# Koellewe/nano-dpow

Measured on AMD Instinct MI355X. Metric: Gnonce/s blake2b-64 per GPU & 8-GPU node; p50 time-to-work at fffffff8, higher is better.
Workload: dtype u64

## Files before the change

### include/nanopow.h

```cpp
#ifndef NANOPOW_H
#define NANOPOW_H

#include <stdint.h>

#ifdef __cplusplus
extern "C" {
#endif

#define NPOW_OK 0
#define NPOW_CANCELLED 1
#define NPOW_EXHAUSTED 2
#define NPOW_PENDING 3
#define NPOW_TOO_LATE 4
#define NPOW_ERR_NOT_INITIALISED (-1)
#define NPOW_ERR_NO_DEVICE (-2)
#define NPOW_ERR_BAD_ARGUMENT (-3)
#define NPOW_ERR_HIP (-4)
#define NPOW_ERR_INVALID_WORK (-5)
#define NPOW_ERR_CAPACITY (-6)
#define NPOW_ERR_INTERNAL (-7)

#define NPOW_ABI_VERSION 7

#define NPOW_RESERVE_MIN 0xfffff00000000000ull
// ... 165 lines not shown
  uint64_t nonces_done;
  uint64_t nonce, value;
  uint64_t launches;
  uint64_t records;
  uint64_t records_max;
  uint64_t room;
} npow_best_info;

int npow_ticket_best(uint64_t ticket, npow_best_info* out);

int npow_submit_best_background(const uint8_t root[32], uint64_t floor, uint64_t start, uint64_t count,
                                uint64_t device_mask, const volatile uint32_t* cancel, uint64_t* ticket);

typedef struct npow_best_hold_info {
  uint32_t size;
  uint32_t background;
  uint64_t launches_cut;
  uint64_t held_us;
} npow_best_hold_info;

int npow_ticket_best_hold(uint64_t ticket, npow_best_hold_info* out);

int npow_submit_sweep_shared(const uint8_t root[32], uint64_t threshold, uint64_t start, uint64_t count,
                             uint64_t device_mask, const volatile uint32_t* cancel, uint64_t* ticket);
int npow_submit_best_shared(const uint8_t root[32], uint64_t floor, uint64_t start, uint64_t count,
                            uint64_t device_mask, const volatile uint32_t* cancel, uint64_t* ticket);

typedef struct npow_range_share_info {
  uint32_t size;
  uint32_t klass;
  uint64_t launches;
  uint64_t launches_cut;
  uint64_t held_us;
  uint64_t moves;
} npow_range_share_info;

int npow_ticket_share(uint64_t ticket, npow_range_share_info* out);

int npow_values(int device, const uint8_t root[32], uint64_t start, uint64_t count, uint64_t* values_out);

int npow_values_path(int device, const uint8_t root[32], uint64_t start, uint64_t count, int path,
                     uint64_t* values_out);

int npow_values_pairs(int device, const uint8_t* roots, const uint64_t* nonces, uint32_t n,
                      uint64_t* values_out);

int npow_set_tuning(uint32_t iters_per_launch, uint32_t poll_interval, uint32_t blocks_per_cu);

int npow_set_pool_tuning(uint32_t budget_us, uint32_t blocks_per_cu);

int npow_device_stats_get(int device, npow_device_stats* out);
int npow_device_stats_get_sized(int device, npow_device_stats* out, uint64_t size);
int npow_device_stats_reset(int device);

const char* npow_version(void);
int npow_abi_version(void);

#ifdef __cplusplus
}
#endif

#endif
```

### nano-dpow_amd/csrc/npow_engine.cpp

```cpp
#include <hip/hip_runtime.h>

#include <pthread.h>
#include <time.h>

#include <algorithm>
#include <cstddef>
#include <exception>
#include <chrono>
#include <cstdio>
#include <cstdlib>
#include <cstring>
#include <deque>
#include <memory>
#include <mutex>
#include <string>
#include <thread>
#include <vector>

#include "npow_host.h"

namespace npow {

namespace {
thread_local std::string t_err;
// ... 475 lines not shown
  out->host_cpu_ms = cpu - d.worker_cpu0_ms;
  out->host_wall_ms = std::chrono::duration<double, std::milli>(std::chrono::steady_clock::now() - d.stats_t0).count();
  out->dead = d.dead ? 1 : 0;
  out->pool_groups = kLsGroups;
  out->early_finishes = d.early;
  out->early_mismatches = d.early_mismatch;
  out->yields = d.yields;
  out->dyn_entries = d.dyn;
  out->kills_relayed = d.kills_relayed;
  out->late_nonces = d.late;
  out->hip_device = d.hip_id;
  out->cu_first = d.cu_first;
  out->idle_ms = d.idle_ms;
  out->idle_gaps = d.idle_gaps;
  out->affinity_checks = d.affinity_checks.load(std::memory_order_relaxed);
  out->affinity_failures = d.affinity_failures.load(std::memory_order_relaxed);
  out->watcher_decisions = d.watcher_decisions;
  out->stale_drains = d.stale_drains;
  out->linger_relays = d.linger_relays;
  out->stale_late = d.stale_late;
  out->stale_missing = d.stale_missing;
  out->stale_gpu_delay_us = d.stale_gpu_delay_us;
  out->linger_ms = d.linger_ms;
  out->promotions = d.promotions;
  return NPOW_OK;
}

int npow_device_stats_get(int device, npow_device_stats* out) try {
  if (!out) return fail(NPOW_ERR_BAD_ARGUMENT, "out is required");
  npow_device_stats full;
  if (int rc = stats_fill(device, &full)) return rc;
  memcpy(out, &full, offsetof(npow_device_stats, kills_relayed));
  return NPOW_OK;
} catch (...) { return guard_exception(); }

int npow_device_stats_get_sized(int device, npow_device_stats* out, uint64_t size) try {
  if (!out || size == 0) return fail(NPOW_ERR_BAD_ARGUMENT, "out and size > 0 are required");
  npow_device_stats full;
  if (int rc = stats_fill(device, &full)) return rc;
  memcpy(out, &full, std::min<uint64_t>(size, sizeof(full)));
  return NPOW_OK;
} catch (...) { return guard_exception(); }

int npow_device_stats_reset(int device) try {
  if (int rc = check_init()) return rc;
  if (device < 0 || device >= (int)g_devs.size()) return fail(NPOW_ERR_BAD_ARGUMENT, "bad device");
  Device& d = *g_devs[device];
  settle_stats(d);
  const double cpu = worker_cpu_ms(d);
  std::lock_guard<std::mutex> g(d.stats_mu);
  d.launches = d.nonces = d.invalid = d.early = d.early_mismatch = d.yields = d.dyn = d.kills_relayed = d.late = 0;
  d.promotions = d.idle_gaps = d.watcher_decisions = d.stale_drains = d.linger_relays = d.stale_late = d.stale_missing = 0;
  d.idle_ms = d.linger_ms = d.stale_gpu_delay_us = 0.0;
  d.kernel_ms = 0.0;
  d.clk_ticks = d.clk_ref_ticks = 0.0;
  d.stats_t0 = std::chrono::steady_clock::now();
  d.worker_cpu0_ms = cpu;
  return NPOW_OK;
} catch (...) { return guard_exception(); }

int npow_search(const uint8_t root[32], uint64_t threshold, uint64_t start, uint64_t device_mask,
                uint64_t max_nonces_per_device, const volatile uint32_t* cancel, uint64_t* nonce_out,
                uint64_t* value_out, uint64_t* nonces_done) try {
  if (int rc = check_init()) return rc;
  if (!root || !nonce_out) return fail(NPOW_ERR_BAD_ARGUMENT, "root and nonce_out are required");
  uint64_t ticket = 0;
  if (int rc = pool_submit(root, threshold, start, device_mask, max_nonces_per_device, cancel, &ticket)) return rc;
  return pool_wait(ticket, -1, nonce_out, value_out, nonces_done);
} catch (...) { return guard_exception(); }

int npow_search_batch(const uint8_t* roots, const uint64_t* thresholds, uint32_t n, uint64_t device_mask,
                      uint64_t max_nonces_per_root, const volatile uint32_t* const* cancel, uint64_t* nonces_out,
                      uint64_t* values_out, int32_t* status_out, uint64_t* nonces_done) try {
  if (int rc = check_init()) return rc;
  if (nonces_done) *nonces_done = 0;
  if (n == 0) return NPOW_OK;
  if (!roots || !thresholds || !nonces_out || !status_out)
    return fail(NPOW_ERR_BAD_ARGUMENT, "roots, thresholds, nonces_out and status_out are required");
  std::vector<uint64_t> tickets(n, 0);
  int err = NPOW_OK;
  std::string err_msg;
  for (uint32_t i = 0; i < n; ++i) {
    const uint8_t* r = roots + 32 * (size_t)i;
    const uint64_t start = host_load_le64(r) ^ host_load_le64(r + 24);
    int rc = pool_submit(r, thresholds[i], start, device_mask, max_nonces_per_root, cancel ? cancel[i] : nullptr,
                         &tickets[i]);
    if (rc) {
      status_out[i] = rc;
      if (err == NPOW_OK) {
        err = rc;
        err_msg = last_error();
      }
    }
  }
  uint64_t total = 0;
  for (uint32_t i = 0; i < n; ++i) {
    if (!tickets[i]) continue;
    uint64_t nonce = 0, value = 0, done = 0;
    const int rc = pool_wait(tickets[i], -1, &nonce, &value, &done);
    total += done;
    status_out[i] = rc;
    if (rc == NPOW_OK) {
      nonces_out[i] = nonce;
      if (values_out) values_out[i] = value;
    } else if (rc < 0 && err == NPOW_OK) {
      err = rc;
      err_msg = last_error();
    }
  }
  if (nonces_done) *nonces_done = total;
  if (err != NPOW_OK) return fail(err, err_msg);
// ... 370 lines not shown
```

### nano-dpow_amd/csrc/npow_host.h

```cpp
#pragma once
#include <hip/hip_runtime.h>
#include <pthread.h>

#include <atomic>
#include <condition_variable>
#include <chrono>
#include <memory>
#include <mutex>
#include <string>
#include <thread>
#include <vector>

#include "../../include/nanopow.h"
#include "npow_blake2b.h"
#include "npow_internal.h"

namespace npow {

int fail(int code, const std::string& msg);
const std::string& last_error();

#define HIPTRY(expr)                                                                        \
  do {                                                                                      \
    hipError_t e_ = (expr);                                                                 \
    if (e_ != hipSuccess)                                                                   \
      return ::npow::fail(NPOW_ERR_HIP, std::string(#expr) + ": " + hipGetErrorString(e_)); \
  } while (0)

constexpr int kEventRing = 4;
static_assert(kEventRing == sizeof(PoolMailbox::clk) / sizeof(PoolMailbox::clk[0]), "one clock record set per ring");

struct Device {
  int id = 0;
  int cpu_threads = 0;
  int hip_id = 0;
  int cus = 0;
  bool time_shared = false;
  int cu_first = -1;
  hipStream_t stream = nullptr;
  DevState* st = nullptr;
  HostMailbox* mb = nullptr;
  HostMailbox* mb_dev = nullptr;
  uint64_t* d_out = nullptr;
  hipEvent_t ev_start[kEventRing] = {};
  hipEvent_t ev_stop[kEventRing] = {};
  std::mutex mu;
  std::atomic<int> tasks_waiting{0};
  PoolDevState* pst = nullptr;
  PoolMailbox* pmb = nullptr;
  PoolMailbox* pmb_dev = nullptr;
  PoolTable* d_tab[kEventRing] = {};
  PoolTable* h_tab[kEventRing] = {};
  unsigned long long* h_done = nullptr;
  hipEvent_t ev_done[kMaxSlots] = {};
  hipStream_t hit_stream = nullptr;
  unsigned long long* h_hit_ring = nullptr;
  unsigned long long* h_hit_n = nullptr;
  uint64_t* h_hits = nullptr;
  std::thread worker;
  std::mutex stats_mu;
  uint64_t launches = 0, nonces = 0, invalid = 0;
  uint64_t early = 0, early_mismatch = 0;
  uint64_t yields = 0, dyn = 0;
  uint64_t linger_ends = 0;
  uint64_t promotions = 0;
  std::atomic<int> counted_inflight{0};
  uint64_t kills_relayed = 0;
  uint64_t late = 0;
  uint64_t watcher_decisions = 0;
  uint64_t stale_drains = 0;
  uint64_t stale_late = 0;
  uint64_t stale_missing = 0;
  double stale_gpu_delay_us = 0.0;
  uint64_t linger_relays = 0;
  double linger_ms = 0.0;
  double idle_ms = 0.0;
  uint64_t idle_gaps = 0;
  std::atomic<bool> worker_busy{false};
  std::atomic<int> active_slots{0};
  std::mutex wake_mu;
  std::condition_variable wake_cv;
  uint64_t wake_seq = 0;
  std::atomic<uint64_t> armed_mask{0};
  std::atomic<uint64_t> armed_gen[kMaxSlots] = {};
  std::atomic<const volatile uint32_t*> armed_cancel[kMaxSlots] = {};
  std::atomic<double> armed_spin_until[kMaxSlots] = {};
  std::mutex armed_mu;
  std::shared_ptr<void> armed_job[kMaxSlots];
  double kernel_ms = 0.0;
  double clk_ticks = 0.0, clk_ref_ticks = 0.0;
  std::chrono::steady_clock::time_point stats_t0 = std::chrono::steady_clock::now();
  double worker_cpu0_ms = 0.0;
  std::atomic<bool> dead{false};
  int dead_code = NPOW_ERR_HIP;
  std::string dead_msg;
  std::atomic<uint64_t> affinity_checks{0}, affinity_failures{0};
  std::mutex cpu_tids_mu;
  std::vector<pthread_t> cpu_tids;
};

extern std::vector<std::unique_ptr<Device>> g_devs;
extern std::atomic<uint32_t> g_iters;
extern std::atomic<uint32_t> g_poll;
extern std::atomic<uint32_t> g_blocks_per_cu;
extern std::atomic<uint32_t> g_budget_us;

inline int grid_of(const Device& d) { return d.cus * (int)g_blocks_per_cu.load(); }
inline int ls_grid(const Device& d) { return d.cus * kLsGroups; }
inline PoolShape pool_shape(const Device& d) { return PoolShape{ls_grid(d)}; }
inline uint32_t poll_mask() {
  uint32_t p = g_poll.load();
  uint32_t m = 1;
  while (m < p) m <<= 1;
  return m - 1;
}

// ... 81 lines not shown
```

### nano-dpow_amd/csrc/npow_internal.h

```cpp
#pragma once
#include <stddef.h>
#include <stdint.h>
#include <hip/hip_runtime.h>

#include "npow_blake2b.h"
#include "npow_weights.h"
#include "npow_claims.h"
#include "npow_dense.h"
#include "npow_hash_asm.inc"
#include "npow_hash_asm_lockstep_ld.inc"

namespace npow {

constexpr int kBlock = 256;
constexpr int kLsWaves = 8;
constexpr int kLsBlock = kLsWaves * 64;
static_assert(kDenseWaves == (uint32_t)kLsWaves, "npow_dense.h: one block per wave of a workgroup");
constexpr int kLsGroups = 4;

enum class Mode : int { kSweep = 1, kValues = 2, kValuesSeq = 3 };

struct LaunchArgs {
  uint64_t u[NPOW_ASM_N_UNIFORMS];
  uint64_t threshold;
// ... 153 lines not shown
  uint64_t t_fin;
  uint64_t t_relay;
  uint64_t t_join;
  uint64_t linger_gen;
  uint64_t stale;
};
static_assert(sizeof(PoolFin) == 64, "one line per slot");
struct alignas(16) PoolFloor {
  uint64_t threshold;
  uint64_t gen;
};
struct alignas(16) PoolReserve {
  uint64_t gen;
  uint64_t nonce;
};
constexpr int kDynEntries = 32;
constexpr int kDynRing = 2 * kDynEntries;
struct alignas(64) PoolDynEntry {
  PoolEntry e;
};
static_assert(sizeof(PoolDynEntry) == 192, "3 cache lines per dynamic entry");
struct PoolMailbox {
  PoolWin win[kMaxSlots];
  PoolFin fin[kMaxSlots];
  PoolDynEntry dyn[kDynRing];
  uint64_t kill[kMaxSlots];
  uint64_t boost[kMaxSlots];
  PoolFloor floor[kMaxSlots];
  PoolReserve reserve[kMaxSlots];
  alignas(64) uint64_t ctl;
  alignas(64) uint64_t kills;
  alignas(64) PoolClk clk[kPoolRing][kClkWaves];
#ifdef NPOW_DIAG_TIMES
  uint64_t diag_join[1024];
#endif
};

struct PoolShape {
  int grid;
  uint32_t units() const { return (uint32_t)grid; }
  uint64_t own(uint32_t e, uint32_t n, uint32_t iters) const {
    return dense_own(units(), n, e, iters);
  }
  uint64_t full(uint32_t iters) const { return dense_full(units(), iters); }
  uint32_t launch_iters(uint32_t iters) const { return iters > 1 ? iters / 2 : 1u; }
};

hipError_t launch_task(Mode mode, int grid, hipStream_t stream, const LaunchArgs& a, DevState* st,
                       HostMailbox* mb, uint64_t* out);
hipError_t launch_pool(hipStream_t stream, int grid, const PoolTable* tab, bool bounded, PoolDevState* st,
                       PoolMailbox* mb);
hipError_t launch_pool_arg(hipStream_t stream, int grid, const PoolTable& host_tab, bool bounded, PoolDevState* st,
                           PoolMailbox* mb);
inline void fill_uniforms(LaunchArgs& a, const RootPrecomp& pre) { npow_asm_uniforms(pre.m, a.u); }

hipError_t launch_pairs(int grid, hipStream_t stream, const uint64_t* roots_words, const uint64_t* nonces,
                        uint32_t n, uint64_t* out);

}
```

### nano-dpow_amd/csrc/npow_kernel.hip

```cpp
#include <hip/hip_runtime.h>
#include <stdint.h>
#include <string.h>

#include "npow_internal.h"

namespace npow {

__device__ __forceinline__ uint64_t pack(uint32_t lo, uint32_t hi) { return ((uint64_t)hi << 32) | lo; }

__device__ __forceinline__ uint64_t rotr32(uint64_t x) {
  return pack((uint32_t)(x >> 32), (uint32_t)x);
}
template <int N>
__device__ __forceinline__ uint64_t rotr_lt32(uint64_t x) {
  const uint32_t lo = (uint32_t)x, hi = (uint32_t)(x >> 32);
  return pack(__builtin_amdgcn_alignbit(hi, lo, N), __builtin_amdgcn_alignbit(lo, hi, N));
}
__device__ __forceinline__ uint64_t rotr63(uint64_t x) {
  const uint32_t lo = (uint32_t)x, hi = (uint32_t)(x >> 32);
  return pack(__builtin_amdgcn_alignbit(lo, hi, 31), __builtin_amdgcn_alignbit(hi, lo, 31));
}

template <int I>
__device__ __forceinline__ uint64_t add_msg(uint64_t a, uint64_t nonce, const uint64_t (&m)[4]) {
// ... 1021 lines not shown
    }
    __syncthreads();
    e = __builtin_amdgcn_readfirstlane(__hip_atomic_load(&s_next, __ATOMIC_RELAXED, __HIP_MEMORY_SCOPE_WORKGROUP));
    ++seg;
  }
  if constexpr (BOUNDED) {
    if (e != kNoEntry || !counted) break;
    __syncthreads();
    if (wv == 0) {
      const uint32_t next = ls2_move_claimed(tab, st, mb, (uint32_t)t_start);
      if (lane == 0) s_next = next;
    }
    __syncthreads();
    e = __builtin_amdgcn_readfirstlane(__hip_atomic_load(&s_next, __ATOMIC_RELAXED, __HIP_MEMORY_SCOPE_WORKGROUP));
    if (e == kNoEntry) break;
    continue;
  }
  if (e != kNoEntry || !tab->linger) break;
  __syncthreads();
  if (wv == 0) {
    const uint32_t next = ls2_linger(tab, st, mb, &s_seen, 0);
    if (lane == 0) s_next = next;
  }
  __syncthreads();
  e = __builtin_amdgcn_readfirstlane(__hip_atomic_load(&s_next, __ATOMIC_RELAXED, __HIP_MEMORY_SCOPE_WORKGROUP));
  if (e == kNoEntry) break;
  }
  if (!counted && wv == 0) ls2_exit(tab, st, mb, G, g);
  clk_end_ls2(tab, mb, t_start, wv);
}

template <bool BOUNDED>
__global__ __launch_bounds__(kLsBlock, 8) void npow_pool_kernel_ls2(const PoolTable* __restrict__ tab,
                                                                   PoolDevState* __restrict__ st,
                                                                   PoolMailbox* __restrict__ mb) {
  uint64_t t_start;
  asm volatile("s_memrealtime %0\n\ts_waitcnt lgkmcnt(0)" : "=s"(t_start) :: "memory");
  clk_begin_lds();
  pool_body_ls2<BOUNDED>(tab, st, mb, t_start);
}

template <bool BOUNDED>
__global__ __launch_bounds__(kLsBlock, 8) void npow_pool_kernel_ls2_arg(const PoolTableArg targ,
                                                                       PoolDevState* __restrict__ st,
                                                                       PoolMailbox* __restrict__ mb) {
  uint64_t t_start;
  asm volatile("s_memrealtime %0\n\ts_waitcnt lgkmcnt(0)" : "=s"(t_start) :: "memory");
  (void)targ;
  const PoolTable* tab = (const PoolTable*)__builtin_amdgcn_kernarg_segment_ptr();
  clk_begin_lds();
  pool_body_ls2<BOUNDED>(tab, st, mb, t_start);
}

hipError_t launch_pool(hipStream_t stream, int grid, const PoolTable* tab, bool bounded, PoolDevState* st,
                       PoolMailbox* mb) {
  if (bounded)
    npow_pool_kernel_ls2<true><<<grid, kLsBlock, 0, stream>>>(tab, st, mb);
  else
    npow_pool_kernel_ls2<false><<<grid, kLsBlock, 0, stream>>>(tab, st, mb);
  return hipGetLastError();
}

hipError_t launch_pool_arg(hipStream_t stream, int grid, const PoolTable& host_tab, bool bounded, PoolDevState* st,
                           PoolMailbox* mb) {
  if (host_tab.n > (uint32_t)kArgEntries) return hipErrorInvalidValue;
  PoolTableArg a;
  memcpy(&a, &host_tab, pool_table_bytes(host_tab.n));
  if (bounded)
    npow_pool_kernel_ls2_arg<true><<<grid, kLsBlock, 0, stream>>>(a, st, mb);
  else
    npow_pool_kernel_ls2_arg<false><<<grid, kLsBlock, 0, stream>>>(a, st, mb);
  return hipGetLastError();
}

__global__ __launch_bounds__(kBlock) void npow_pairs_kernel(const uint64_t* __restrict__ roots_words,
                                                            const uint64_t* __restrict__ nonces, uint32_t n,
                                                            uint64_t* __restrict__ out) {
  const uint32_t i = blockIdx.x * kBlock + threadIdx.x;
  if (i >= n) return;
  uint64_t m[4];
#pragma unroll
  for (int k = 0; k < 4; ++k) m[k] = roots_words[4 * (size_t)i + k];
  out[i] = work_value_full(nonces[i], m);
}

hipError_t launch_task(Mode mode, int grid, hipStream_t stream, const LaunchArgs& a, DevState* st,
                       HostMailbox* mb, uint64_t* out) {
  switch (mode) {
    case Mode::kSweep:
      npow_sweep_kernel_ls2<<<grid, kLsBlock, 0, stream>>>(a, st, mb, out);
      break;
    case Mode::kValues:
      npow_values_kernel_ls2<<<grid, kLsBlock, 0, stream>>>(a, st, out);
      break;
    case Mode::kValuesSeq:
      npow_values_kernel_seq<<<grid, kBlock, 0, stream>>>(a, st, out);
      break;
  }
  return hipGetLastError();
}

hipError_t launch_pairs(int grid, hipStream_t stream, const uint64_t* roots_words, const uint64_t* nonces,
                        uint32_t n, uint64_t* out) {
  npow_pairs_kernel<<<grid, kBlock, 0, stream>>>(roots_words, nonces, n, out);
  return hipGetLastError();
}
// ... 3 lines not shown
```

### nano-dpow_amd/csrc/npow_pool.cpp

```cpp
#include <hip/hip_runtime.h>
#include <sys/prctl.h>

#include <algorithm>
#include <chrono>
#include <cmath>
#include <condition_variable>
#include <deque>
#include <mutex>
#include <string>
#include <thread>
#include <vector>

#include "npow_pool_impl.h"

namespace npow {
namespace {

constexpr double kYieldMinUs = 1500.0;
constexpr int kYieldMaxLive = 8;
constexpr int kIdleSpinUs = 2000;
constexpr double kPrelaunchUs = 2000.0;
constexpr double kDynMinUs = 3000.0;
constexpr double kFreshSpinUs = 400.0;
constexpr int kInvalidStreakMax = 3;
// ... 904 lines not shown
  bool fg = foreground_live(-1);
  for (uint32_t e = 0; e < n && !fg; ++e) fg = !slots_[idx[e]].job->background && !slots_[idx[e]].job->shared;
  const double t = now_us();
  uint32_t m = 0;
  for (uint32_t e = 0; e < n; ++e) {
    Slot& sl = slots_[idx[e]];
    if (!sl.job->held_class()) {
      idx[m++] = idx[e];
      continue;
    }
    JobDev& jd = sl.job->dev[sl.k];
    if (fg) {
      if (!sl.held) jd.held_since = t;
      sl.held = true;
      continue;
    }
    if (sl.held) {
      jd.held_us += t - jd.held_since;
      jd.held_since = 0;
      sl.held = false;
    }
    idx[m++] = idx[e];
  }
  return m;
}

int Worker::launch(bool empty_linger) {
  if (q_.size() >= 2 || d_.dead) return NPOW_OK;
  if (q_.size() == 1 && g_budget_us.load() > 0 && budget_left_us() > kPrelaunchUs && live_slot()) return NPOW_OK;
  uint32_t n = 0;
  int idx[kMaxSlots];
  bool claimed = false;
  for (int s = 0; s < kMaxSlots; ++s)
    if (slots_[s].state == SlotState::kActive && !slots_[s].no_more) {
      idx[n++] = s;
      claimed = claimed || slots_[s].job->held_class();
    }
  if (claimed) n = hold_out(idx, n);
  if (n == 0 && !empty_linger) return NPOW_OK;
  if (!live_slot()) end_linger();
  PoolTable& t = *d_.h_tab[ring_];
  bool bounded = false;
  build_table(t, idx, n, &bounded);
  if (n == 0 && !t.linger) return NPOW_OK;
  const PoolShape sh = pool_shape(d_);
  const int r = ring_;
  ring_ = (ring_ + 1) % kEventRing;
  const size_t bytes = pool_table_bytes(n);
  DEVCHECK(d_, "pool launch");
  if (faults().hip_dev == d_.id && seq_ > faults().hip_after)
    return fail(NPOW_ERR_HIP, "injected launch failure (NANOPOW_FAULT_HIP)");
  if (!collect_.empty())
    HIPTRY(hipMemsetAsync(&d_.pst->hits[r & 1], 0, offsetof(PoolHits, rec), d_.stream));
  if (n <= (uint32_t)kArgEntries) {
    HIPTRY(hipEventRecord(d_.ev_start[r], d_.stream));
    HIPTRY(launch_pool_arg(d_.stream, sh.grid, t, bounded, d_.pst, d_.pmb_dev));
  } else {
    HIPTRY(hipMemcpyAsync(d_.d_tab[r], d_.h_tab[r], bytes, hipMemcpyHostToDevice, d_.stream));
    HIPTRY(hipEventRecord(d_.ev_start[r], d_.stream));
    HIPTRY(launch_pool(d_.stream, sh.grid, d_.d_tab[r], bounded, d_.pst, d_.pmb_dev));
  }
  if (!collect_.empty())
    HIPTRY(hipMemcpyAsync(d_.h_hit_ring + (size_t)r * (offsetof(PoolHits, rec) / sizeof(unsigned long long)),
                          &d_.pst->hits[r & 1], offsetof(PoolHits, rec), hipMemcpyDeviceToHost, d_.stream));
  HIPTRY(hipEventRecord(d_.ev_stop[r], d_.stream));
  if (q_.empty()) front_start_ = std::chrono::steady_clock::now();
  NPOW_DBGT("nanopow[%d]: launch %llu n=%u linger %u wsum %u (weights halved %u times) yield_base %llx slots:", d_.id,
            (unsigned long long)seq_, n, t.linger, t.wsum ? t.wsum : pool_claimed_pad_sum(t.pad), t.wdown, (unsigned long long)t.yield_base);
  for (uint32_t e = 0; e < n; ++e) NPOW_DBG(" %d/g%llu", idx[e], (unsigned long long)t.e[e].gen);
  NPOW_DBG("\n");
  q_.push_back({seq_, r, (uint32_t)ctl_, t.yield_base, t.counted != 0, t.linger != 0, t.wdown, bounded, collect_});
  publish_counted();
  return NPOW_OK;
}

int Worker::queue_readbacks() {
  constexpr size_t row = kPoolDoneShards * 8;
  DEVCHECK(d_, "pool read-back");
  for (int s = 0; s < kMaxSlots; ++s) {
    Slot& sl = slots_[s];
    if (sl.state != SlotState::kDraining || sl.readback || sl.no_readback) continue;
    if (!g_readback_always && !d_.dead) {
      if (sl.early) {
        if (++early_count_ % kVerifyEvery != 0) {
          sl.no_readback = true;
          continue;
        }
      } else if (!sl.fin_seen && sl.stop_us > 0 && !sl.requeue && !sl.inflight.empty() &&
                 now_us() - sl.stop_us < g_linger_us) {
        continue;
      }
    }
    HIPTRY(hipMemcpyAsync(d_.h_done + (size_t)s * row, &d_.pst->done[s][0], row * sizeof(unsigned long long),
                          hipMemcpyDeviceToHost, d_.stream));
    HIPTRY(hipEventRecord(d_.ev_done[s], d_.stream));
    sl.readback = true;
  }
  return NPOW_OK;
}

void Worker::trace_launch(const PoolInflight& f, uint64_t g0, uint64_t g1) {
  float ev = 0.f;
  if (hipEventElapsedTime(&ev, d_.ev_start[f.ring], d_.ev_stop[f.ring]) == hipSuccess)
    fprintf(stderr, "nanopow-launch dev %d launch %llu: events %.1f clock waves %.1f us, start %.1f us after the "
            "previous end\n", d_.id, (unsigned long long)f.seq, ev * 1e3, (double)(g1 - g0) / 100.0,
            prev_g1_ ? ((double)g0 - (double)prev_g1_) / 100.0 : -1.0);
  prev_g1_ = g1;
// ... 502 lines not shown
```

### nano-dpow_amd/csrc/npow_pool_impl.h

```cpp
#pragma once
#include <cstdio>
#include <cstdlib>
#include <cstring>

#include "npow_pool.h"

namespace npow {

inline const char* env_str(const char* name, const char* dflt) { const char* e = getenv(name); return e ? e : dflt; }
inline double env_num(const char* name, double dflt) { const char* e = getenv(name); return e ? atof(e) : dflt; }
inline const double g_poll_us = env_num("NANOPOW_POLL_US", 50.0);
inline const bool g_debug = getenv("NANOPOW_DEBUG") != nullptr;
inline const int g_linger_env = getenv("NANOPOW_LINGER") ? (getenv("NANOPOW_LINGER")[0] == '0' ? 0 : 1) : -1;
inline const uint32_t g_linger_p = [] {
  uint32_t p = (uint32_t)atoi(env_str("NANOPOW_LINGER_P", "0")), q = 1;
  while (p && q < p) q <<= 1;
  return p ? q : 0u;
}();
inline const double g_linger_us = env_num("NANOPOW_LINGER_US", 1000.0);
inline const bool g_readback_always = strcmp(env_str("NANOPOW_READBACK", ""), "always") == 0;
inline const bool g_watcher_on = strcmp(env_str("NANOPOW_WATCHER", "1"), "0") != 0;
inline const double g_watch_nap_us = env_num("NANOPOW_WATCH_NAP_US", 20.0);
inline const bool g_trace_lat = getenv("NANOPOW_TRACE_LATENCY") != nullptr;
inline const bool g_trace_steps = getenv("NANOPOW_TRACE_STEPS") != nullptr;
inline const bool g_wait_spin = env_str("NANOPOW_WAIT_SPIN", "1")[0] != '0';

struct Faults {
  uint64_t invalid_mask = 0;
  int hip_dev = -1;
  uint64_t hip_after = 0;
  bool retarget_blind = false;
  bool no_moves = false;
};
const Faults& faults();

#define NPOW_DBG(...) \
  do { if (g_debug) fprintf(stderr, __VA_ARGS__); } while (0)
#define NPOW_DBGT(...) \
  do { if (g_debug) fprintf(stderr, "[%.3f] ", now_us() * 1e-3), fprintf(stderr, __VA_ARGS__); } while (0)

void wake_worker(Device& d);


inline void mb_kill(Device& d, int s, uint64_t gen) {
  __atomic_store_n(&d.pmb->kill[s], gen, __ATOMIC_RELEASE);
  __atomic_fetch_add(&d.pmb->kills, 1ull, __ATOMIC_RELEASE);
}
inline void mb_boost(Device& d, int s, uint64_t gen, uint32_t weight) {
  __atomic_store_n(&d.pmb->boost[s], pool_boost_word(gen, pool_wsh(weight)), __ATOMIC_RELEASE);
  __atomic_fetch_add(&d.pmb->kills, 1ull << 32, __ATOMIC_RELEASE);
}
inline void mb_floor(Device& d, int s, uint64_t gen, uint64_t threshold) {
  PoolFloor& f = d.pmb->floor[s];
  if (__atomic_load_n(&f.gen, __ATOMIC_RELAXED) != gen) {
    __atomic_store_n(&f.threshold, threshold, __ATOMIC_RELAXED);
    __atomic_store_n(&f.gen, gen, __ATOMIC_RELEASE);
  } else {
    __atomic_store_n(&f.threshold, threshold, __ATOMIC_RELEASE);
  }
}
inline void mb_yield(Device& d, uint64_t& ctl) {
  ctl += 1ull << 32;
  __atomic_store_n(&d.pmb->ctl, ctl, __ATOMIC_RELEASE);
}
template <class F>
inline void for_each_gpu_slot(Job& j, F&& f) {
// ... 23 lines not shown
```

### nano-dpow_amd/nanopow/_lib.py

```python
from __future__ import annotations

import ctypes
import os
import threading
import time
from dataclasses import dataclass
from typing import List, Optional, Sequence, Tuple

_HERE = os.path.dirname(os.path.abspath(__file__))
LIB_PATH = os.environ.get("NANOPOW_LIB", os.path.join(_HERE, "libnanopow.so"))

NPOW_OK = 0
NPOW_CANCELLED = 1
NPOW_EXHAUSTED = 2
NPOW_PENDING = 3
NPOW_TOO_LATE = 4
NPOW_ERR_NOT_INITIALISED = -1
NPOW_ERR_NO_DEVICE = -2
NPOW_ERR_BAD_ARGUMENT = -3
NPOW_ERR_HIP = -4
NPOW_ERR_INVALID_WORK = -5
NPOW_ERR_CAPACITY = -6
NPOW_ERR_INTERNAL = -7

NPOW_ABI_VERSION = 7
NPOW_RESERVE_MIN = 0xfffff00000000000
NPOW_PATH_SEARCH = 0
NPOW_PATH_SEQ = 1
NPOW_PATH_GENERIC = 2

NPOW_SWEEP_JOB_HITS = 1 << 20

M64 = (1 << 64) - 1

EXPORTED_SYMBOLS = (
    "npow_init", "npow_shutdown", "npow_last_error", "npow_work_value", "npow_search",
    "npow_search_batch", "npow_sweep", "npow_values", "npow_values_pairs", "npow_set_tuning",
    "npow_device_stats_get", "npow_device_stats_reset", "npow_version",
    "npow_submit", "npow_wait", "npow_cancel", "npow_pool_config", "npow_pool_status",
    "npow_set_pool_tuning", "npow_values_path", "npow_wait_info", "npow_device_stats_get_sized",
    "npow_abi_version", "npow_config_cpu_threads", "npow_wait_result", "npow_submit_weighted",
    "npow_promote", "npow_retarget", "npow_submit_background", "npow_ticket_background",
    "npow_submit_reserve", "npow_ticket_reserve", "npow_relax", "npow_submit_sweep", "npow_wait_sweep",
    "npow_submit_sweep_background", "npow_ticket_sweep", "npow_submit_best", "npow_wait_best", "npow_ticket_best",
    "npow_submit_best_background", "npow_ticket_best_hold",
    "npow_submit_sweep_shared", "npow_submit_best_shared", "npow_ticket_share",
)


class NanoPowError(RuntimeError):
    def __init__(self, code: int, message: str):
        super().__init__(f"nanopow error {code}: {message}")
        self.code = code
        self.message = message


class DeviceStats(ctypes.Structure):
    _fields_ = [
        ("launches", ctypes.c_uint64),
        ("nonces", ctypes.c_uint64),
        ("kernel_ms", ctypes.c_double),
        ("invalid_work", ctypes.c_uint64),
        ("cus", ctypes.c_int32),
        ("grid", ctypes.c_int32),
        ("clock_mhz", ctypes.c_double),
        ("host_cpu_ms", ctypes.c_double),
        ("host_wall_ms", ctypes.c_double),
        ("dead", ctypes.c_int32),
        ("pool_groups", ctypes.c_int32),
        ("early_finishes", ctypes.c_uint64),
        ("early_mismatches", ctypes.c_uint64),
        ("yields", ctypes.c_uint64),
        ("dyn_entries", ctypes.c_uint64),
        ("kills_relayed", ctypes.c_uint64),
        ("late_nonces", ctypes.c_uint64),
        ("hip_device", ctypes.c_int32),
        ("cu_first", ctypes.c_int32),
        ("idle_ms", ctypes.c_double),
        ("idle_gaps", ctypes.c_uint64),
        ("affinity_checks", ctypes.c_uint64),
        ("affinity_failures", ctypes.c_uint64),
        ("watcher_decisions", ctypes.c_uint64),
        ("stale_drains", ctypes.c_uint64),
        ("linger_ms", ctypes.c_double),
        ("linger_relays", ctypes.c_uint64),
        ("stale_late", ctypes.c_uint64),
        ("stale_missing", ctypes.c_uint64),
        ("stale_gpu_delay_us", ctypes.c_double),
        ("promotions", ctypes.c_uint64),
    ]


class SearchInfo(ctypes.Structure):
    _fields_ = [
        ("size", ctypes.c_uint32),
        ("status", ctypes.c_int32),
        ("nonce", ctypes.c_uint64),
        ("value", ctypes.c_uint64),
        ("nonces_done", ctypes.c_uint64),
# ... 169 lines not shown
                               "(or __graft_entry__.build())")
        lib = ctypes.CDLL(path)
        u8p = ctypes.c_char_p
        u64, u32 = ctypes.c_uint64, ctypes.c_uint32
        pu64 = ctypes.POINTER(ctypes.c_uint64)
        p = ctypes.c_void_p
        lib.npow_init.argtypes = [ctypes.POINTER(ctypes.c_int)]
        lib.npow_init.restype = ctypes.c_int
        lib.npow_shutdown.argtypes = []
        lib.npow_shutdown.restype = None
        lib.npow_last_error.argtypes = []
        lib.npow_last_error.restype = ctypes.c_char_p
        lib.npow_version.argtypes = []
        lib.npow_version.restype = ctypes.c_char_p
        lib.npow_work_value.argtypes = [u8p, u64]
        lib.npow_work_value.restype = u64
        lib.npow_search.argtypes = [u8p, u64, u64, u64, u64, p, pu64, pu64, pu64]
        lib.npow_search.restype = ctypes.c_int
        lib.npow_search_batch.argtypes = [u8p, p, u32, u64, u64, p, p, p, p, pu64]
        lib.npow_search_batch.restype = ctypes.c_int
        lib.npow_sweep.argtypes = [u8p, u64, u64, u64, u64, p, p, u64, pu64]
        lib.npow_sweep.restype = ctypes.c_int
        lib.npow_values.argtypes = [ctypes.c_int, u8p, u64, u64, p]
        lib.npow_values.restype = ctypes.c_int
        lib.npow_values_pairs.argtypes = [ctypes.c_int, u8p, p, u32, p]
        lib.npow_values_pairs.restype = ctypes.c_int
        lib.npow_set_tuning.argtypes = [u32, u32, u32]
        lib.npow_set_tuning.restype = ctypes.c_int
        lib.npow_device_stats_get.argtypes = [ctypes.c_int, ctypes.POINTER(DeviceStats)]
        lib.npow_device_stats_get.restype = ctypes.c_int
        lib.npow_device_stats_reset.argtypes = [ctypes.c_int]
        lib.npow_device_stats_reset.restype = ctypes.c_int
        lib.npow_submit.argtypes = [u8p, u64, u64, u64, u64, p, pu64]
        lib.npow_submit.restype = ctypes.c_int
        lib.npow_wait.argtypes = [u64, ctypes.c_int64, pu64, pu64, pu64]
        lib.npow_wait.restype = ctypes.c_int
        lib.npow_cancel.argtypes = [u64]
        lib.npow_cancel.restype = ctypes.c_int
        lib.npow_pool_config.argtypes = [u32]
        lib.npow_pool_config.restype = ctypes.c_int
        lib.npow_pool_status.argtypes = [ctypes.POINTER(ctypes.c_uint32), ctypes.POINTER(ctypes.c_uint32)]
        lib.npow_pool_status.restype = ctypes.c_int
        lib.npow_set_pool_tuning.argtypes = [u32, u32]
        lib.npow_set_pool_tuning.restype = ctypes.c_int
        if hasattr(lib, "npow_abi_version"):
            lib.npow_values_path.argtypes = [ctypes.c_int, u8p, u64, u64, ctypes.c_int, p]
            lib.npow_values_path.restype = ctypes.c_int
            lib.npow_wait_info.argtypes = [u64, ctypes.c_int64, ctypes.POINTER(SearchInfo)]
            lib.npow_wait_info.restype = ctypes.c_int
            lib.npow_device_stats_get_sized.argtypes = [ctypes.c_int, ctypes.POINTER(DeviceStats), u64]
            lib.npow_device_stats_get_sized.restype = ctypes.c_int
            lib.npow_abi_version.argtypes = []
            lib.npow_abi_version.restype = ctypes.c_int
        if hasattr(lib, "npow_config_cpu_threads"):
            lib.npow_config_cpu_threads.argtypes = [u32]
            lib.npow_config_cpu_threads.restype = ctypes.c_int
            lib.npow_wait_result.argtypes = [u64, ctypes.c_int64, pu64, pu64]
            lib.npow_wait_result.restype = ctypes.c_int
        if hasattr(lib, "npow_submit_weighted"):
            lib.npow_submit_weighted.argtypes = [u8p, u64, u64, u64, u64, p, u32, pu64]
            lib.npow_submit_weighted.restype = ctypes.c_int
        if hasattr(lib, "npow_promote"):
            lib.npow_promote.argtypes = [u64, u32]
            lib.npow_promote.restype = ctypes.c_int
        if hasattr(lib, "npow_retarget"):
            lib.npow_retarget.argtypes = [u64, u64]
            lib.npow_retarget.restype = ctypes.c_int
        if hasattr(lib, "npow_submit_background"):
            lib.npow_submit_background.argtypes = [u8p, u64, u64, u64, p, pu64]
            lib.npow_submit_background.restype = ctypes.c_int
            lib.npow_ticket_background.argtypes = [u64, ctypes.POINTER(ctypes.c_uint32)]
            lib.npow_ticket_background.restype = ctypes.c_int
        if hasattr(lib, "npow_submit_reserve"):
            lib.npow_submit_reserve.argtypes = [u8p, u64, u64, u64, u64, p, u32, u32, pu64]
            lib.npow_submit_reserve.restype = ctypes.c_int
            lib.npow_ticket_reserve.argtypes = [u64, ctypes.POINTER(ReserveInfo)]
            lib.npow_ticket_reserve.restype = ctypes.c_int
            lib.npow_relax.argtypes = [u64, u64, ctypes.POINTER(ctypes.c_uint32)]
            lib.npow_relax.restype = ctypes.c_int
        if hasattr(lib, "npow_submit_sweep"):
            lib.npow_submit_sweep.argtypes = [u8p, u64, u64, u64, u64, p, pu64]
            lib.npow_submit_sweep.restype = ctypes.c_int
            lib.npow_wait_sweep.argtypes = [u64, ctypes.c_int64, p, u64, pu64, pu64]
            lib.npow_wait_sweep.restype = ctypes.c_int
        if hasattr(lib, "npow_submit_sweep_background"):
            lib.npow_submit_sweep_background.argtypes = [u8p, u64, u64, u64, u64, p, pu64]
            lib.npow_submit_sweep_background.restype = ctypes.c_int
            lib.npow_ticket_sweep.argtypes = [u64, ctypes.POINTER(_SweepInfoStruct)]
            lib.npow_ticket_sweep.restype = ctypes.c_int
        if hasattr(lib, "npow_submit_best"):
            lib.npow_submit_best.argtypes = [u8p, u64, u64, u64, u64, p, pu64]
            lib.npow_submit_best.restype = ctypes.c_int
            lib.npow_wait_best.argtypes = [u64, ctypes.c_int64, pu64, pu64, pu64]
            lib.npow_wait_best.restype = ctypes.c_int
            lib.npow_ticket_best.argtypes = [u64, ctypes.POINTER(_BestInfoStruct)]
            lib.npow_ticket_best.restype = ctypes.c_int
        if hasattr(lib, "npow_submit_best_background"):
            lib.npow_submit_best_background.argtypes = [u8p, u64, u64, u64, u64, p, pu64]
            lib.npow_submit_best_background.restype = ctypes.c_int
            lib.npow_ticket_best_hold.argtypes = [u64, ctypes.POINTER(_BestHoldStruct)]
            lib.npow_ticket_best_hold.restype = ctypes.c_int
        if hasattr(lib, "npow_submit_sweep_shared"):
            for f in (lib.npow_submit_sweep_shared, lib.npow_submit_best_shared):
                f.argtypes = [u8p, u64, u64, u64, u64, p, pu64]
                f.restype = ctypes.c_int
            lib.npow_ticket_share.argtypes = [u64, ctypes.POINTER(_RangeShareStruct)]
# ... 423 lines not shown
                                       cancel.address if cancel else None, ctypes.byref(t)), self.lib)
        return BestTicket(self, t.value, cancel)

    def sweep(self, root: bytes, threshold: int, start: int, count: int, device_mask: int = 0,
              cap: int = 1 << 16, cancel: Optional[CancelToken] = None) -> List[int]:
        r = self.sweep_result(root, threshold, start, count, device_mask, cap, cancel)
        if r.status != NPOW_OK:
            raise NanoPowError(r.status, f"sweep cancelled after {r.total} hits: the hit set is partial")
        return r.hits

    def values(self, root: bytes, start: int, count: int, device: int = 0, path: Optional[int] = None) -> List[int]:
        out = (ctypes.c_uint64 * max(count, 1))()
        if path is None:
            rc = self.lib.npow_values(device, _root(root), start & M64, count, ctypes.addressof(out))
        else:
            rc = self.lib.npow_values_path(device, _root(root), start & M64, count, path, ctypes.addressof(out))
        _check(rc, self.lib)
        return list(out[:count])

    def values_array(self, root: bytes, start: int, count: int, device: int = 0, path: int = NPOW_PATH_SEARCH):
        import numpy as np
        out = np.empty(max(count, 1), dtype=np.uint64)
        _check(self.lib.npow_values_path(device, _root(root), start & M64, count, path, out.ctypes.data), self.lib)
        return out[:count]

    def values_pairs(self, roots: Sequence[bytes], nonces: Sequence[int], device: int = 0) -> List[int]:
        n = len(nonces)
        if len(roots) != n:
            raise ValueError(f"{len(roots)} roots for {n} nonces")
        rb = b"".join(_root(r) for r in roots)
        nn = (ctypes.c_uint64 * max(n, 1))(*[x & M64 for x in nonces])
        out = (ctypes.c_uint64 * max(n, 1))()
        _check(self.lib.npow_values_pairs(device, rb, ctypes.addressof(nn), n, ctypes.addressof(out)), self.lib)
        return list(out[:n])

    def set_tuning(self, iters_per_launch: int = 0, poll_interval: int = 0, blocks_per_cu: int = 0) -> None:
        _check(self.lib.npow_set_tuning(iters_per_launch, poll_interval, blocks_per_cu), self.lib)

    def set_pool_tuning(self, budget_us: Optional[int] = None, blocks_per_cu: int = 0) -> None:
        _check(self.lib.npow_set_pool_tuning(0xffffffff if budget_us is None else budget_us, blocks_per_cu),
               self.lib)

    def set_launch_budget(self, budget_us: int) -> None:
        self.set_pool_tuning(budget_us=budget_us)

    def stats(self, device: int = 0) -> DeviceStats:
        s = DeviceStats()
        if hasattr(self.lib, "npow_device_stats_get_sized"):
            _check(self.lib.npow_device_stats_get_sized(device, ctypes.byref(s), ctypes.sizeof(s)), self.lib)
        else:
            _check(self.lib.npow_device_stats_get(device, ctypes.byref(s)), self.lib)
        return s

    def abi_version(self) -> int:
        return int(self.lib.npow_abi_version())

    def reset_stats(self, device: int = 0) -> None:
        _check(self.lib.npow_device_stats_reset(device), self.lib)

    def version(self) -> str:
        return self.lib.npow_version().decode()


_engine: Optional[Engine] = None
_engine_lock = threading.Lock()


def engine(cpu_threads: int = 0) -> Engine:
    global _engine
    with _engine_lock:
        if _engine is None:
            _engine = Engine(cpu_threads=cpu_threads)
        return _engine
```

Baseline: 35.07.

## Add specialized single-entry solo kernel for unbounded pool launches

Adds a dedicated kernel for the common case of a single unbounded, non-counted, non-background pool entry. The kernel drops the multi-entry table scan and bounded bookkeeping, and reloads kernarg pointers only on rare paths (hits, polls) to lower register pressure in the hot hash loop. It is enabled by default, can be disabled via NANOPOW_SOLO=0, and exposes a solo launch counter through a new API and a Python binding. It adds a second kernel to keep consistent with the pool semantics, which is a risk for correctness in edge cases.

```diff
diff --git a/include/nanopow.h b/include/nanopow.h
--- a/include/nanopow.h
+++ b/include/nanopow.h
@@ -241,6 +241,7 @@
 int npow_device_stats_get(int device, npow_device_stats* out);
 int npow_device_stats_get_sized(int device, npow_device_stats* out, uint64_t size);
 int npow_device_stats_reset(int device);
+int64_t npow_device_solo_launches(int device);
 
 const char* npow_version(void);
 int npow_abi_version(void);
diff --git a/nano-dpow_amd/csrc/npow_engine.cpp b/nano-dpow_amd/csrc/npow_engine.cpp
--- a/nano-dpow_amd/csrc/npow_engine.cpp
+++ b/nano-dpow_amd/csrc/npow_engine.cpp
@@ -551,11 +551,21 @@
   d.launches = d.nonces = d.invalid = d.early = d.early_mismatch = d.yields = d.dyn = d.kills_relayed = d.late = 0;
   d.promotions = d.idle_gaps = d.watcher_decisions = d.stale_drains = d.linger_relays = d.stale_late = d.stale_missing = 0;
   d.idle_ms = d.linger_ms = d.stale_gpu_delay_us = 0.0;
+  d.solo_launches = 0;
   d.kernel_ms = 0.0;
   d.clk_ticks = d.clk_ref_ticks = 0.0;
   d.stats_t0 = std::chrono::steady_clock::now();
   d.worker_cpu0_ms = cpu;
   return NPOW_OK;
+} catch (...) { return guard_exception(); }
+
+int64_t npow_device_solo_launches(int device) try {
+  if (int rc = check_init()) return rc;
+  if (device < 0 || device >= (int)g_devs.size()) return fail(NPOW_ERR_BAD_ARGUMENT, "bad device");
+  Device& d = *g_devs[device];
+  settle_stats(d);
+  std::lock_guard<std::mutex> g(d.stats_mu);
+  return (int64_t)d.solo_launches;
 } catch (...) { return guard_exception(); }
 
 int npow_search(const uint8_t root[32], uint64_t threshold, uint64_t start, uint64_t device_mask,
diff --git a/nano-dpow_amd/csrc/npow_host.h b/nano-dpow_amd/csrc/npow_host.h
--- a/nano-dpow_amd/csrc/npow_host.h
+++ b/nano-dpow_amd/csrc/npow_host.h
@@ -62,6 +62,7 @@
   uint64_t launches = 0, nonces = 0, invalid = 0;
   uint64_t early = 0, early_mismatch = 0;
   uint64_t yields = 0, dyn = 0;
+  uint64_t solo_launches = 0;
   uint64_t linger_ends = 0;
   uint64_t promotions = 0;
   std::atomic<int> counted_inflight{0};
diff --git a/nano-dpow_amd/csrc/npow_internal.h b/nano-dpow_amd/csrc/npow_internal.h
--- a/nano-dpow_amd/csrc/npow_internal.h
+++ b/nano-dpow_amd/csrc/npow_internal.h
@@ -229,6 +229,7 @@
                        PoolMailbox* mb);
 hipError_t launch_pool_arg(hipStream_t stream, int grid, const PoolTable& host_tab, bool bounded, PoolDevState* st,
                            PoolMailbox* mb);
+hipError_t launch_solo_arg(hipStream_t stream, int grid, const PoolTable& host_tab, PoolDevState* st, PoolMailbox* mb);
 inline void fill_uniforms(LaunchArgs& a, const RootPrecomp& pre) { npow_asm_uniforms(pre.m, a.u); }
 
 hipError_t launch_pairs(int grid, hipStream_t stream, const uint64_t* roots_words, const uint64_t* nonces,
diff --git a/nano-dpow_amd/csrc/npow_kernel.hip b/nano-dpow_amd/csrc/npow_kernel.hip
--- a/nano-dpow_amd/csrc/npow_kernel.hip
+++ b/nano-dpow_amd/csrc/npow_kernel.hip
@@ -1097,6 +1097,164 @@
   pool_body_ls2<BOUNDED>(tab, st, mb, t_start);
 }
 
+__shared__ uint64_t s_solo_t0;
+struct SoloKernarg {
+  PoolTableArg t;
+  PoolDevState* st;
+  PoolMailbox* mb;
+};
+static_assert(offsetof(SoloKernarg, st) == sizeof(PoolTableArg) && sizeof(PoolTableArg) % 8 == 0, "as the ABI lays them");
+typedef const __attribute__((address_space(4))) SoloKernarg ConstSoloKernarg;
+__device__ __forceinline__ ConstSoloKernarg* solo_args() {
+  ConstSoloKernarg* ka = (ConstSoloKernarg*)__builtin_amdgcn_kernarg_segment_ptr();
+  asm volatile("" : "+s"(ka));
+  return ka;
+}
+__global__ __launch_bounds__(kLsBlock, 8) void npow_solo_kernel(const PoolTableArg targ, PoolDevState* __restrict__ st,
+                                                               PoolMailbox* __restrict__ mb) {
+  uint64_t t_start;
+  asm volatile("s_memrealtime %0\n\ts_waitcnt lgkmcnt(0)" : "=s"(t_start) :: "memory");
+  (void)targ;
+  const PoolTable* tab = (const PoolTable*)__builtin_amdgcn_kernarg_segment_ptr();
+  clk_begin_lds();
+  __shared__ uint32_t s_stop;
+  __shared__ uint32_t s_flag[kLsWaves];
+  __shared__ uint32_t s_live, s_seen;
+  const uint32_t lane = threadIdx.x & 63;
+  const uint32_t wv = __builtin_amdgcn_readfirstlane(threadIdx.x >> 6);
+  const uint32_t g = blockIdx.x, G = gridDim.x;
+  const uint32_t t0 = (uint32_t)t_start;
+  ConstEntry* const ce = (ConstEntry*)(uintptr_t)&tab->e[0];
+  if (threadIdx.x == 0) {
+    s_stop = ~0u;
+    s_seen = 0;
+    s_over = 0;
+    s_solo_t0 = t_start;
+  }
+  if (wv == 0) {
+    const uint32_t live = load_dead(st, ce->slot) < ce->gen ? 1u : 0u;
+    if (lane == 0) s_live = live;
+  }
+  __syncthreads();
+  uint32_t it = 0;
+  if (__builtin_amdgcn_readfirstlane(__hip_atomic_load(&s_live, __ATOMIC_RELAXED, __HIP_MEMORY_SCOPE_WORKGROUP))) {
+    const uint64_t* const up = tab->e[0].u;
+    const uint32_t iters = tab->iters, poll_mask = tab->poll_mask, budget = tab->budget;
+    const uint32_t gen_lo = (uint32_t)ce->gen;
+    uint64_t thr = ce->reserve;
+    unsigned long long* const dead_p = &st->slot[ce->slot].dead;
+    const uint32_t step = (G * kLsWaves) << 6;
+    uint64_t nonce = ce->base + ((uint64_t)(g * kLsWaves + wv) << 6) + lane;
+    uint32_t pc = g * kLsWaves + wv;
+    while (it < iters) {
+      const uint32_t verdict = __hip_atomic_load(&s_stop, __ATOMIC_RELAXED, __HIP_MEMORY_SCOPE_WORKGROUP);
+      uint64_t dead;
+      asm volatile("" : "=v"(dead));
+      if (wv == 0) dead = __hip_atomic_load(dead_p, __ATOMIC_RELAXED, __HIP_MEMORY_SCOPE_AGENT);
+      const uint32_t v = (uint32_t)__builtin_amdgcn_readfirstlane(verdict);
+      if (v != ~0u && (v >> 2) <= it) break;
+      const uint32_t it0 = it;
+      const uint32_t pc0 = pc;
+      const uint64_t value = npow_asm_work_value_lockstep_ld(nonce, up);
+      ++it;
+      pc += kPollStride;
+      uint32_t why = 0u;
+      if (__builtin_expect(__builtin_amdgcn_uicmp((uint32_t)(value >> 32), (uint32_t)(thr >> 32), 35) != 0, 0)) {
+        uint64_t hits = __ballot(value >= thr);
+        if (hits != 0) {
+          ConstSoloKernarg* const ka = solo_args();
+          PoolDevState* const st = ka->st;
+          PoolMailbox* const mb = ka->mb;
+          ConstEntry* const ce = (ConstEntry*)&ka->t.e[0];
+          const uint32_t wslot = ce->slot;
+          const uint64_t wgen = ce->gen;
+          PoolFloor* const fl = &mb->floor[wslot];
+          const uint64_t fgen = __hip_atomic_load(&fl->gen, __ATOMIC_RELAXED, __HIP_MEMORY_SCOPE_SYSTEM);
+          ls2_complete();
+          const uint64_t ethr = ce->threshold;
+          uint64_t cur = ethr;
+          if (uni64(fgen) == wgen) {
+            const uint64_t fthr = __hip_atomic_load(&fl->threshold, __ATOMIC_RELAXED, __HIP_MEMORY_SCOPE_SYSTEM);
+            ls2_complete();
+            cur = uni64(fthr);
+          }
+          const bool armed = ce->reserve != ethr;
+          if (cur > thr) {
+            if (!armed) thr = cur;
+            const uint64_t keep = hits & __ballot(value >= cur);
+            const uint64_t stale = hits & ~keep & __ballot(value >= ethr);
+            if (stale != 0 && lane == 0)
+              atomicAdd(&st->done[wslot][(blockIdx.x % kPoolDoneShards) * 8 + kStaleWord],
+                        (unsigned long long)__builtin_popcountll(stale));
+            uint64_t cand = hits & ~keep & ~stale;
+            hits = keep;
+            if (cand != 0) {
+              uint64_t bv = 0, bn = 0;
+              do {
+                const int cl = __builtin_ctzll(cand);
+                cand &= cand - 1;
+                const uint64_t cv = readlane64(value, cl);
+                if (cv >= bv) {
+                  bv = cv;
+                  bn = readlane64(nonce, cl);
+                }
+              } while (cand != 0);
+              if (lane == 0) ls2_publish_reserve(st, mb, wslot, wgen, bn, bv);
+            }
+          }
+          if (hits != 0) {
+            why = 2u;
+            const int wl = __builtin_ctzll(hits);
+            const uint64_t wn = readlane64(nonce, wl), wval = readlane64(value, wl);
+            if (lane == 0) ls2_publish_win(st, mb, wslot, wgen, wn, wval);
+          }
+        }
+      }
+      if (__builtin_expect((pc0 & poll_mask) == 0, 0)) {
+        ConstSoloKernarg* const ka = solo_args();
+        if (lane == 0) s_flag[wv] = ls2_poll((const PoolTable*)(uintptr_t)ka, ka->st, ka->mb, 0, &s_seen);
+        lds_drain();
+        const uint32_t p = __builtin_amdgcn_readfirstlane(
+            __hip_atomic_load(&s_flag[wv], __ATOMIC_RELAXED, __HIP_MEMORY_SCOPE_WAVEFRONT));
+        why = (p & 2u) ? 2u : (why ? why : (p ? 3u : 0u));
+      }
+      if (wv == 0 && __builtin_expect(__builtin_amdgcn_uicmp((uint32_t)dead, gen_lo, 32) != 0, 0)) {
+        if (__ballot(dead == solo_args()->t.e[0].gen) != 0) why = 1u;
+      }
+      const bool late = budget && (it0 & 3u) == 0 && (uint32_t)__builtin_amdgcn_s_memrealtime() - t0 >= budget;
+      if (__builtin_expect(why != 0 || late, 0)) {
+        if (lane == 0)
+          __hip_atomic_fetch_min(&s_stop, (it << 2) | (late ? 0u : why), __ATOMIC_RELAXED, __HIP_MEMORY_SCOPE_WORKGROUP);
+        lds_drain();
+      }
+      nonce += step;
+      __builtin_amdgcn_s_barrier();
+    }
+    __syncthreads();
+    if (wv == 0) {
+      const uint32_t sum = it * 64u * kLsWaves;
+      const uint32_t v = __builtin_amdgcn_readfirstlane(
+          __hip_atomic_load(&s_stop, __ATOMIC_RELAXED, __HIP_MEMORY_SCOPE_WORKGROUP));
+      const uint32_t kind = v != ~0u && (v >> 2) == it ? (v & 3u) : 0u;
+      uint32_t late_n = kind == 1u ? 64u * kLsWaves : 0u;
+      late_n = late_n < sum ? late_n : sum;
+      ls2_leave_wave(st, mb, ce->slot, ce->gen, sum, late_n, false);
+    }
+  }
+  if (wv == 0) ls2_exit(tab, st, mb, G, g);
+  if (wv == 0 && g < (uint32_t)kClkWaves)
+    clk_end_ls2(tab, mb, uni64(__hip_atomic_load(&s_solo_t0, __ATOMIC_RELAXED, __HIP_MEMORY_SCOPE_WORKGROUP)), wv);
+}
+
+hipError_t launch_solo_arg(hipStream_t stream, int grid, const PoolTable& host_tab, PoolDevState* st,
+                           PoolMailbox* mb) {
+  if (host_tab.n != 1u) return hipErrorInvalidValue;
+  PoolTableArg a;
+  memcpy(&a, &host_tab, pool_table_bytes(1));
+  npow_solo_kernel<<<grid, kLsBlock, 0, stream>>>(a, st, mb);
+  return hipGetLastError();
+}
+
 hipError_t launch_pool(hipStream_t stream, int grid, const PoolTable* tab, bool bounded, PoolDevState* st,
                        PoolMailbox* mb) {
   if (bounded)
diff --git a/nano-dpow_amd/csrc/npow_pool.cpp b/nano-dpow_amd/csrc/npow_pool.cpp
--- a/nano-dpow_amd/csrc/npow_pool.cpp
+++ b/nano-dpow_amd/csrc/npow_pool.cpp
@@ -980,7 +980,13 @@
     return fail(NPOW_ERR_HIP, "injected launch failure (NANOPOW_FAULT_HIP)");
   if (!collect_.empty())
     HIPTRY(hipMemsetAsync(&d_.pst->hits[r & 1], 0, offsetof(PoolHits, rec), d_.stream));
-  if (n <= (uint32_t)kArgEntries) {
+  const bool solo = g_solo_env && n == 1 && !bounded && !t.counted && !t.linger && t.e[0].bounded == 0 && !t.e[0].bg;
+  if (solo) {
+    HIPTRY(hipEventRecord(d_.ev_start[r], d_.stream));
+    HIPTRY(launch_solo_arg(d_.stream, sh.grid, t, d_.pst, d_.pmb_dev));
+    std::lock_guard<std::mutex> sg(d_.stats_mu);
+    d_.solo_launches++;
+  } else if (n <= (uint32_t)kArgEntries) {
     HIPTRY(hipEventRecord(d_.ev_start[r], d_.stream));
     HIPTRY(launch_pool_arg(d_.stream, sh.grid, t, bounded, d_.pst, d_.pmb_dev));
   } else {
diff --git a/nano-dpow_amd/csrc/npow_pool_impl.h b/nano-dpow_amd/csrc/npow_pool_impl.h
--- a/nano-dpow_amd/csrc/npow_pool_impl.h
+++ b/nano-dpow_amd/csrc/npow_pool_impl.h
@@ -12,6 +12,7 @@
 inline const double g_poll_us = env_num("NANOPOW_POLL_US", 50.0);
 inline const bool g_debug = getenv("NANOPOW_DEBUG") != nullptr;
 inline const int g_linger_env = getenv("NANOPOW_LINGER") ? (getenv("NANOPOW_LINGER")[0] == '0' ? 0 : 1) : -1;
+inline const bool g_solo_env = !(getenv("NANOPOW_SOLO") && getenv("NANOPOW_SOLO")[0] == '0');
 inline const uint32_t g_linger_p = [] {
   uint32_t p = (uint32_t)atoi(env_str("NANOPOW_LINGER_P", "0")), q = 1;
   while (p && q < p) q <<= 1;
diff --git a/nano-dpow_amd/nanopow/_lib.py b/nano-dpow_amd/nanopow/_lib.py
--- a/nano-dpow_amd/nanopow/_lib.py
+++ b/nano-dpow_amd/nanopow/_lib.py
@@ -45,6 +45,7 @@
     "npow_submit_sweep_background", "npow_ticket_sweep", "npow_submit_best", "npow_wait_best", "npow_ticket_best",
     "npow_submit_best_background", "npow_ticket_best_hold",
     "npow_submit_sweep_shared", "npow_submit_best_shared", "npow_ticket_share",
+    "npow_device_solo_launches",
 )
 
 
@@ -320,6 +321,9 @@
             lib.npow_device_stats_get_sized.restype = ctypes.c_int
             lib.npow_abi_version.argtypes = []
             lib.npow_abi_version.restype = ctypes.c_int
+        if hasattr(lib, "npow_device_solo_launches"):
+            lib.npow_device_solo_launches.argtypes = [ctypes.c_int]
+            lib.npow_device_solo_launches.restype = ctypes.c_int64
         if hasattr(lib, "npow_config_cpu_threads"):
             lib.npow_config_cpu_threads.argtypes = [u32]
             lib.npow_config_cpu_threads.restype = ctypes.c_int
@@ -849,6 +853,12 @@
             _check(self.lib.npow_device_stats_get(device, ctypes.byref(s)), self.lib)
         return s
 
+    def solo_launches(self, device: int = 0) -> int:
+        n = int(self.lib.npow_device_solo_launches(device))
+        if n < 0:
+            _check(n, self.lib)
+        return n
+
     def abi_version(self) -> int:
         return int(self.lib.npow_abi_version())
 
```

New measurement: 35.14, median of 6. No clear change (+0.2%).
